# v-iashin/Synchformer

Measured on AMD Instinct MI355X. Metric: clips/sec (14-seg offset pred), higher is better.
Workload: dtype bf16; 1 GPU; BASELINE configs[1]: batched offset inference, configs/sync.yaml model (237.5M params, random-init), uint8 224x224 frames + 16 kHz waveform segments resident in HBM; RGB + log-mel front-ends and the full forward to 21-way logits inside the timed step; clips_per_gpu=16, segments=14, seg_chunk=224, hip_graph=False, parallelism=replicas x1

## Files before the change

synchformer_amd/csrc/sf_qkv_time2.hip:

```cpp
#include "sf_common.h"
#include <type_traits>
#include <stdlib.h>
#include "../../include/synchformer_hip.h"

#define QT2_NP 196
#define QT2_TP 24
#define QT2_ROWS 192
#define QT2_D 768
#define QT2_A_BYTES (QT2_ROWS * 128)
#define QT2_W_PART (128 * 128)
#define QT2_STAGE (QT2_A_BYTES + 3 * QT2_W_PART)
#ifndef QT2_ABL_HALF
#define QT2_ABL_HALF 0
#endif
#define QT2_ARR (QT2_ROWS * 128)
#define QT2_CB_OFF (6 * QT2_ARR)
#define QT2_BIAS_OFF (QT2_CB_OFF + 6 * 2048)
#define QT2_LAND_OFF (QT2_BIAS_OFF + 1536)
#define QT2_CBX_OFF QT2_CB_OFF
#define QT2_ZROW_OFF (QT2_CB_OFF + 6 * 128)
#define QT2_SC_OFF (QT2_CB_OFF + 1024)
#define QT2_SC_BYTES 2304
#define QT2_MASK_OFF (QT2_LAND_OFF + 768)
#define QT2_LDS (160 * 1024)
#define QT2_NPART 33
#ifndef QT2_ABL
#define QT2_ABL 0
#endif

struct Qt2Args {
  const bf16_t* X; int64_t ldx;
  const bf16_t* W; int64_t ldw;
  const float* bias;
  const bf16_t* side; int64_t lds_;
  bf16_t* out; int64_t ldo;
  float* cls_part;
  int64_t seq_rows;
  uint32_t n_rt;
  uint32_t pair_chunk;
  float scale;
  uint32_t stagger;
  const uint8_t* key_keep = nullptr;
  const uint8_t* sX = nullptr; int64_t ldsx = 0;
  const uint8_t* sW = nullptr; int64_t ldsw = 0;
  uint8_t* out_q = nullptr; int64_t ldq = 0; uint8_t* out_s = nullptr; int64_t splane = 0;
};
typedef __attribute__((ext_vector_type(8))) int qt2_i32x8;

typedef short qt2_s4 __attribute__((ext_vector_type(4)));
typedef __attribute__((address_space(3))) qt2_s4 qt2_lds_s4;

__device__ __forceinline__ void qt2_dma1(uint32_t voff, const void* sbase, uint32_t lds) {
  uint32_t keep;
  asm volatile("s_mov_b32 %0, m0\n\ts_mov_b32 m0, %3\n\ts_nop 0\n\tglobal_load_lds_dwordx4 %1, %2\n\ts_mov_b32 m0, %0"
               : "=&s"(keep) : "v"(voff), "s"(sbase), "s"(lds) : "memory");
}
__device__ __forceinline__ void qt2_dma_dword_addr(const void* gaddr, uint32_t lds) {
  uint32_t keep;
  asm volatile("s_mov_b32 %0, m0\n\ts_mov_b32 m0, %2\n\ts_nop 0\n\tglobal_load_lds_dword %1, off\n\ts_mov_b32 m0, %0"
               : "=&s"(keep) : "v"(gaddr), "s"(lds) : "memory");
}
template <int N>
__device__ __forceinline__ void qt2_wait_vmcnt() {
  asm volatile("" ::: "memory");
  __builtin_amdgcn_s_waitcnt((N & 0xF) | (0x7 << 4) | (0xF << 8) | ((N >> 4) << 14));
}
__device__ __forceinline__ void qt2_barrier() {
  asm volatile("" ::: "memory");
  __builtin_amdgcn_s_barrier();
  asm volatile("" ::: "memory");
}
__device__ __forceinline__ uint32_t qt2_lds_addr(const void* p) { return (uint32_t)(uintptr_t)(__attribute__((address_space(3))) const char*)p; }
__device__ __forceinline__ int qt2_arr_off(int row, int chunk) { return row * 128 + ((chunk ^ (((row >> 3) + row) & 7)) << 4); }

template <int V> using qt2_ic = std::integral_constant<int, V>;

template <bool MASK, bool MX = false>
__device__ __forceinline__ void qkv_time2_attn_body(const Qt2Args& p) {
  constexpr int ESZ = MX ? 1 : 2;
  extern __shared__ __attribute__((aligned(16))) char smem[];
  const int tid = threadIdx.x, lane = tid & 63;
  const int wave = __builtin_amdgcn_readfirstlane(tid >> 6);
  const int wm = wave >> 2, wn = wave & 3;
  const int hi = lane >> 5;

  const uint32_t xcd = blockIdx.x & 7u, li = blockIdx.x >> 3, per_xcd_blocks = gridDim.x >> 3;
  const uint32_t r8 = (p.n_rt + 7u) >> 3;
  const uint32_t rt0 = min(xcd * r8, p.n_rt), rt1 = min(rt0 + r8, p.n_rt);
  const uint32_t hc = p.pair_chunk, chunk_tiles = (rt1 - rt0) * hc, t_end = (rt1 - rt0) * 6u;
  uint32_t t = li;
  if (t >= t_end) return;
  for (uint32_t i = 0, n = ((li / hc) * 8u + xcd) * p.stagger; i < n; ++i) __builtin_amdgcn_s_sleep(32);

  uint32_t voff_a = 0, voff_w[3] = {0, 0, 0}, sc_voff = 0, cls_voff = 0;
  const int sc_seg = wave % 3;
  const int sc_lanes = sc_seg == 0 ? 48 : (sc_seg == 1 ? 64 : 32);
  const uint32_t a8 = (uint32_t)(8 * p.ldx * ESZ), w8 = (uint32_t)(8 * p.ldw * ESZ);
  const uint32_t lds0 = __builtin_amdgcn_readfirstlane(qt2_lds_addr(smem));
  const uint32_t lds_a_w = __builtin_amdgcn_readfirstlane(lds0 + wave * 3072);
  const uint32_t lds_w_w = __builtin_amdgcn_readfirstlane(lds0 + QT2_A_BYTES + wave * 2048);

  for (int x = tid; x < (MX ? 1024 : 6 * 2048) / 16; x += 512) *reinterpret_cast<uint4*>(smem + QT2_CB_OFF + x * 16) = make_uint4(0u, 0u, 0u, 0u);
  qt2_barrier();

  const char* xbase; const char* wbase;
  int64_t seq; int tb, hp;
  auto set_tile = [&](uint32_t tt) {
    const uint32_t c = tt / chunk_tiles, r = tt - c * chunk_tiles;
    const uint32_t rt = rt0 + r / hc;
    hp = (int)(c * hc + r % hc);
    seq = rt / 9u; tb = (int)(rt - (uint32_t)seq * 9u);
    xbase = reinterpret_cast<const char*>(p.X) + (seq * p.seq_rows + 1 + (int64_t)tb * QT2_TP) * p.ldx * ESZ;
    wbase = reinterpret_cast<const char*>(p.W) + (int64_t)hp * 128 * p.ldw * ESZ;
  };
  auto derive_offsets = [&]() {
    int dtid = threadIdx.x;
    asm volatile("" : "+v"(dtid));
    const int dl = dtid & 63;
    {
      const int r = wave * 3 * 8 + (dl >> 3);
      voff_a = (uint32_t)((int64_t)(wave * QT2_NP + (dl >> 3)) * p.ldx * ESZ + ((((dl & 7) ^ ((r >> 1) & 7))) << 4));
    }
#pragma unroll
    for (int j = 0; j < 3; ++j) {
      const int pr = wave * 2 * 8 + (dl >> 3);
      const int c = (pr >> 5) * 96 + j * 32 + (pr & 31);
      const int hd = c / 192, within = c - hd * 192;
      const int grow = (within >> 6) * QT2_D + hd * 64 + (within & 63);
      voff_w[j] = (uint32_t)((int64_t)grow * p.ldw * ESZ + ((((dl & 7) ^ ((pr >> 1) & 7))) << 4));
    }
    { const int ch = dl & 7, w3 = (dl >> 3) % 3, hd = (dl >> 3) / 3; cls_voff = (uint32_t)((w3 * QT2_D + hd * 64 + ch * 8) * 2); }
    if (MX) {
      if (sc_seg == 0) sc_voff = (uint32_t)((dl / 6) * QT2_NP * 4 + (dl % 6) * 16);
      else {
        const int L = (sc_seg == 1 ? 0 : 64) + dl, run = L >> 3, j = run >> 2, wnp = run & 3;
        const int c = wnp * 96 + j * 32 + (L & 7) * 4;
        const int hd = c / 192, within = c - hd * 192;
        sc_voff = (uint32_t)(((within >> 6) * QT2_D + hd * 64 + (within & 63)) * 4);
      }
    }
  };
  const uint32_t sc_lds = __builtin_amdgcn_readfirstlane(lds0 + QT2_SC_OFF + (sc_seg == 0 ? 0 : (sc_seg == 1 ? 768 : 768 + 1024)));
  auto issue_sc = [&](int kt) {
    const char* base = sc_seg == 0 ? reinterpret_cast<const char*>(p.sX) + (int64_t)kt * p.ldsx + (seq * p.seq_rows + 1 + (int64_t)tb * QT2_TP) * 4
                                   : reinterpret_cast<const char*>(p.sW) + (int64_t)kt * p.ldsw + (int64_t)hp * 512;
    if (lane < sc_lanes) qt2_dma1(sc_voff, base, sc_lds + (kt & 1) * QT2_SC_BYTES);
  };
  auto issue_a = [&](int pc, int S, int kt) {
    qt2_dma1(((pc & 1) ? (voff_a ^ 64u) : voff_a) + (uint32_t)pc * a8, xbase + kt * 128, lds_a_w + S * QT2_STAGE + pc * 1024);
  };
  auto issue_w = [&](int j, int S, int kt) {
    qt2_dma1(voff_w[j], wbase + kt * 128, lds_w_w + S * QT2_STAGE + j * QT2_W_PART);
    qt2_dma1((voff_w[j] ^ 64u) + w8, wbase + kt * 128, lds_w_w + S * QT2_STAGE + j * QT2_W_PART + 1024);
  };

  constexpr int nk = MX ? QT2_D / 128 : QT2_D / 64;
  const float sc2 = p.scale * 1.44269504088896f;
  uint32_t tcount = 0;
  auto cb_ptr = [&](int blk, int h, int row, int chunk) -> const char* {
    if (!MX) return smem + QT2_CB_OFF + (blk + h) * 2048 + qt2_arr_off(row, chunk);
    return smem + (row == 0 ? QT2_CBX_OFF + (blk + h) * 128 : QT2_ZROW_OFF) + (chunk << 4);
  };

  for (;;) {
    set_tile(t);
    const bool main_item = tb < 8;
    if (main_item) {
      derive_offsets();
      if (wave < 6) {
        if (p.bias) qt2_dma_dword_addr(p.bias + (wave % 3) * QT2_D + (hp * 2 + wave / 3) * 64 + lane, lds0 + QT2_BIAS_OFF + wave * 256);
      } else if (wave == 7) {
        if (lane < 48) qt2_dma1(cls_voff, reinterpret_cast<const char*>(p.side + seq * 33 * p.lds_ + hp * 128), lds0 + QT2_LAND_OFF);
      }
      if (MX) issue_sc(0);
      issue_w(0, 0, 0); issue_a(0, 0, 0);
      issue_w(1, 0, 0); issue_a(1, 0, 0); issue_a(2, 0, 0);
      issue_w(2, 0, 0);
      issue_w(0, 1, 1); issue_a(0, 1, 1);
      qt2_wait_vmcnt<5>();
      qt2_barrier();

      f32x16 acc[3][3];
      {
        const float* bs = reinterpret_cast<const float*>(smem + QT2_BIAS_OFF);
#pragma unroll
        for (int j = 0; j < 3; ++j)
#pragma unroll
          for (int g = 0; g < 4; ++g) {
            const float4 b4 = p.bias ? *reinterpret_cast<const float4*>(bs + wn * 96 + j * 32 + g * 8 + hi * 4) : make_float4(0.f, 0.f, 0.f, 0.f);
#pragma unroll
            for (int i = 0; i < 3; ++i) { acc[j][i][g * 4 + 0] = b4.x; acc[j][i][g * 4 + 1] = b4.y; acc[j][i][g * 4 + 2] = b4.z; acc[j][i][g * 4 + 3] = b4.w; }
          }
      }
      {
        int fo[4], fs_x = 0, fs_w = 0, shi = 0;
        {
          int ptid = threadIdx.x;
          asm volatile("" : "+v"(ptid));
          const int pl31 = ptid & 31, phi = (ptid & 63) >> 5;
#pragma unroll
          for (int kk = 0; kk < 4; ++kk) fo[kk] = pl31 * 128 + (((kk * 2 + phi) ^ ((pl31 >> 1) & 7)) << 4);
          if (MX) { fs_x = QT2_SC_OFF + (wm * 96 + pl31) * 4; fs_w = QT2_SC_OFF + 768 + (wn * 32 + pl31) * 4; shi = phi * 8; }
        }
        const int a_base = wm * 96 * 128, w_base = QT2_A_BYTES + wn * 32 * 128;
        union Qt2Frag { bf16x8 h[2]; qt2_i32x8 v; };
        Qt2Frag xf[3][2], wf[2];
        uint32_t sx[3] = {0u, 0u, 0u}, sw = 0u;
        auto read_w = [&](const char* st, int j, int par) {
#pragma unroll
          for (int kk = 0; kk < 4; ++kk) wf[kk >> 1].h[kk & 1] = *reinterpret_cast<const bf16x8*>(st + w_base + j * QT2_W_PART + fo[kk]);
          if (MX) sw = *reinterpret_cast<const uint32_t*>(smem + fs_w + j * 512 + par * QT2_SC_BYTES) >> shi;
        };
        auto mma = [&](auto Jc) {
          constexpr int J = decltype(Jc)::value;
          __builtin_amdgcn_s_setprio(1);
          if constexpr (MX) {
#pragma unroll
            for (int k2 = 0; k2 < 2; ++k2) {
#pragma unroll
              for (int i = 0; i < 3; ++i) {
                if (k2 == 0) acc[J][i] = __builtin_amdgcn_mfma_scale_f32_32x32x64_f8f6f4(wf[0].v, xf[i][0].v, acc[J][i], 0 , 0 , 0, (int)sw, 0, (int)sx[i]);
                else acc[J][i] = __builtin_amdgcn_mfma_scale_f32_32x32x64_f8f6f4(wf[1].v, xf[i][1].v, acc[J][i], 0, 0, 2, (int)sw, 2, (int)sx[i]);
              }
            }
          } else
          if (!(QT2_ABL & 2)) {
#pragma unroll
            for (int kk = 0; kk < 4; ++kk)
#pragma unroll
              for (int i = 0; i < 3; ++i) acc[J][i] = __builtin_amdgcn_mfma_f32_32x32x16_bf16(wf[kk >> 1].h[kk & 1], xf[i][kk >> 1].h[kk & 1], acc[J][i], 0, 0, 0);
          } else asm volatile("" :: "v"(wf[0].v), "v"(wf[1].v), "v"(xf[0][0].v), "v"(xf[2][1].v));
          asm volatile("" : "+v"(acc[J][0]), "+v"(acc[J][1]), "+v"(acc[J][2]));
          __builtin_amdgcn_s_setprio(0);
        };
        auto ktile = [&](auto Sc, int kt, bool ld1, bool ld2) {
          constexpr int S = decltype(Sc)::value;
          const char* st = smem + S * QT2_STAGE;
#pragma unroll
          for (int i = 0; i < 3; ++i)
#pragma unroll
            for (int kk = 0; kk < 4; ++kk) xf[i][kk >> 1].h[kk & 1] = *reinterpret_cast<const bf16x8*>(st + a_base + i * 4096 + fo[kk]);
          read_w(st, 0, S);
          if (MX) {
#pragma unroll
            for (int i = 0; i < 3; ++i) sx[i] = *reinterpret_cast<const uint32_t*>(smem + fs_x + i * 128 + S * QT2_SC_BYTES) >> shi;
          }
          __builtin_amdgcn_sched_barrier(0);
          if (ld1) { issue_w(1, S ^ 1, kt + 1); issue_a(1, S ^ 1, kt + 1); issue_a(2, S ^ 1, kt + 1); }
          qt2_barrier();
          __builtin_amdgcn_sched_barrier(0);
          mma(qt2_ic<0>{});
          __builtin_amdgcn_sched_barrier(0);
          qt2_barrier();
          read_w(st, 1, S);
          __builtin_amdgcn_sched_barrier(0);
          if (ld1) { if (MX) issue_sc(kt + 1); issue_w(2, S ^ 1, kt + 1); if (MX) qt2_wait_vmcnt<10>(); else qt2_wait_vmcnt<9>(); } else qt2_wait_vmcnt<0>();
          qt2_barrier();
          __builtin_amdgcn_sched_barrier(0);
          mma(qt2_ic<1>{});
          __builtin_amdgcn_sched_barrier(0);
          qt2_barrier();
          read_w(st, 2, S);
          __builtin_amdgcn_sched_barrier(0);
          if (ld2) { issue_w(0, S, kt + 2); issue_a(0, S, kt + 2); qt2_wait_vmcnt<5>(); }
          else if (ld1) qt2_wait_vmcnt<2>();
          else qt2_wait_vmcnt<0>();
          qt2_barrier();
          __builtin_amdgcn_sched_barrier(0);
          mma(qt2_ic<2>{});
          __builtin_amdgcn_sched_barrier(0);
          qt2_barrier();
        };
        if (wm == 1) qt2_barrier();
#pragma unroll 1
        for (int kt = 0; kt < nk; kt += 2) {
          ktile(qt2_ic<0>{}, kt, true, kt + 2 < nk);
          ktile(qt2_ic<1>{}, kt + 1, kt + 2 < nk, kt + 3 < nk);
        }
        if (wm == 0) qt2_barrier();
      }

      {
        int etid = threadIdx.x;
        asm volatile("" : "+v"(etid));
        const int el31 = etid & 31, ehi = (etid & 63) >> 5;
        uint8_t kflag = 1;
        if (MASK && etid < QT2_ROWS + 1) {
          const int fr = etid / QT2_TP, pl = etid - fr * QT2_TP;
          kflag = etid == QT2_ROWS ? p.key_keep[seq * p.seq_rows] : p.key_keep[seq * p.seq_rows + 1 + (int64_t)fr * QT2_NP + tb * QT2_TP + pl];
        }
        int rowp[3];
#pragma unroll
        for (int i = 0; i < 3; ++i) { const int R = wm * 96 + i * 32 + el31, fr = R / QT2_TP; rowp[i] = (R - fr * QT2_TP) * 8 + fr; }
#pragma unroll
        for (int j = 0; j < 3; ++j) {
          const int cb = (wn * 3 + j) * 32;
          const int hd = cb / 192, within = cb - hd * 192, which = within >> 6, feat0 = within & 63;
          const int arr = hd * 3 * QT2_ARR + (which == 1 ? 0 : (which == 2 ? QT2_ARR : 2 * QT2_ARR));
#pragma unroll
          for (int i = 0; i < 3; ++i) {
#pragma unroll
            for (int g = 0; g < 4; ++g) {
              uint2 w;
              w.x = pack_bf2(acc[j][i][g * 4 + 0], acc[j][i][g * 4 + 1]);
              w.y = pack_bf2(acc[j][i][g * 4 + 2], acc[j][i][g * 4 + 3]);
#if QT2_ABL_HALF
              *reinterpret_cast<uint2*>(smem + arr + qt2_arr_off(rowp[i], (feat0 >> 3) + g) + (ehi ^ ((el31 >> 3) & 1)) * 8) = w;
#else
              *reinterpret_cast<uint2*>(smem + arr + qt2_arr_off(rowp[i], (feat0 >> 3) + g) + ehi * 8) = w;
#endif
            }
          }
        }
        if (etid < 48) {
          const int ch = etid & 7, w3 = (etid >> 3) % 3, hd = (etid >> 3) / 3;
          const uint4 sv = *reinterpret_cast<const uint4*>(smem + QT2_LAND_OFF + etid * 16);
          *reinterpret_cast<uint4*>(const_cast<char*>(cb_ptr(w3 == 1 ? 0 : (w3 == 2 ? 2 : 4), hd, 0, ch))) = sv;
        }
        if (MASK && etid < QT2_ROWS + 1) {
          const int fr = etid / QT2_TP, pl = etid - fr * QT2_TP;
          reinterpret_cast<float*>(smem + QT2_MASK_OFF)[etid == QT2_ROWS ? QT2_ROWS : pl * 8 + fr] = kflag ? 0.f : -INFINITY;
        }
        qt2_barrier();
      }
    } else {
      int stid = threadIdx.x;
      asm volatile("" : "+v"(stid));
      uint4 sv[3], cv = make_uint4(0u, 0u, 0u, 0u);
#pragma unroll
      for (int e = 0; e < 3; ++e) {
        const int x = stid + e * 512, ch = x & 7, rr = (x >> 3) & 31, w3 = (x >> 8) % 3, hd = (x >> 8) / 3;
        sv[e] = *reinterpret_cast<const uint4*>(p.side + (seq * 33 + 1 + (rr & 7) * 4 + (rr >> 3)) * p.lds_ + w3 * QT2_D + (hp * 2 + hd) * 64 + ch * 8);
      }
      if (stid < 48) {
        const int ch = stid & 7, w3 = (stid >> 3) % 3, hd = (stid >> 3) / 3;
        cv = *reinterpret_cast<const uint4*>(p.side + seq * 33 * p.lds_ + w3 * QT2_D + (hp * 2 + hd) * 64 + ch * 8);
      }
#pragma unroll
      for (int e = 0; e < 3; ++e) {
        const int x = stid + e * 512, ch = x & 7, rr = (x >> 3) & 31, w3 = (x >> 8) % 3, hd = (x >> 8) / 3;
        *reinterpret_cast<uint4*>(smem + hd * 3 * QT2_ARR + (w3 == 1 ? 0 : (w3 == 2 ? QT2_ARR : 2 * QT2_ARR)) + qt2_arr_off(rr, ch)) = sv[e];
      }
      if (stid < 48) {
        const int ch = stid & 7, w3 = (stid >> 3) % 3, hd = (stid >> 3) / 3;
        *reinterpret_cast<uint4*>(const_cast<char*>(cb_ptr(w3 == 1 ? 0 : (w3 == 2 ? 2 : 4), hd, 0, ch))) = cv;
      }
      if (MASK && stid >= 64 && stid < 64 + 33) {
        const int r = stid - 64;
        const uint8_t kf = r == 32 ? p.key_keep[seq * p.seq_rows] : p.key_keep[seq * p.seq_rows + 1 + (int64_t)(r & 7) * QT2_NP + QT2_ROWS + (r >> 3)];
        reinterpret_cast<float*>(smem + QT2_MASK_OFF)[r == 32 ? QT2_ROWS : r] = kf ? 0.f : -INFINITY;
      }
      qt2_barrier();
    }

    if (!(QT2_ABL & 1)) {
      int atid = threadIdx.x;
      asm volatile("" : "+v"(atid));
      const int alane = atid & 63, fr_ = alane & 15, fg = alane >> 4;
      const int krow = fg * 4 + (fr_ >> 2), c1 = (fr_ & 3) >> 1, hb = (fr_ & 1) * 8;
      const int64_t orow0 = seq * p.seq_rows + 1 + (main_item ? tb * QT2_TP : QT2_ROWS);
      auto patch_units = [&](auto NUc, const int u0, const int ustep) {
        constexpr int NU = decltype(NUc)::value;
        const char* k_lds[NU];
        int qt[NU], hh_[NU];
        f32x4 s0[NU], s1[NU];
#pragma unroll
        for (int e = 0; e < NU; ++e) {
          const int u = u0 + e * ustep, h = u >= 12 ? 1 : 0;
          qt[e] = u - 12 * h;
          k_lds[e] = smem + h * 3 * QT2_ARR;
          hh_[e] = h;
          s0[e] = f32x4{0.f, 0.f, 0.f, 0.f}; s1[e] = f32x4{0.f, 0.f, 0.f, 0.f};
          if (MASK) {
            const float4 mk = *reinterpret_cast<const float4*>(smem + QT2_MASK_OFF + (qt[e] * 16 + fg * 4) * 4);
            s0[e] = f32x4{mk.x, mk.y, mk.z, mk.w};
            s1[e][0] = reinterpret_cast<const float*>(smem + QT2_MASK_OFF)[QT2_ROWS];
          }
        }
#pragma unroll
        for (int ks = 0; ks < 2; ++ks)
#pragma unroll
          for (int e = 0; e < NU; ++e) {
            const bf16x8 qf = *reinterpret_cast<const bf16x8*>(k_lds[e] + 2 * QT2_ARR + qt2_arr_off(qt[e] * 16 + fr_, ks * 4 + fg));
            const bf16x8 kf = *reinterpret_cast<const bf16x8*>(k_lds[e] + qt2_arr_off(qt[e] * 16 + fr_, ks * 4 + fg));
            const bf16x8 cf = *reinterpret_cast<const bf16x8*>(cb_ptr(0, hh_[e], fr_, ks * 4 + fg));
            s0[e] = __builtin_amdgcn_mfma_f32_16x16x32_bf16(kf, qf, s0[e], 0, 0, 0);
            s1[e] = __builtin_amdgcn_mfma_f32_16x16x32_bf16(cf, qf, s1[e], 0, 0, 0);
          }
        const bool own = (fg >> 1) == (fr_ >> 3);
        float m[NU], l[NU], pc[NU];
#pragma unroll
        for (int e = 0; e < NU; ++e) {
          m[e] = fg == 0 ? s1[e][0] : -INFINITY;
#pragma unroll
          for (int r = 0; r < 4; ++r) { s0[e][r] = own ? s0[e][r] : -INFINITY; m[e] = fmaxf(m[e], s0[e][r]); }
        }
#pragma unroll
        for (int e = 0; e < NU; ++e) m[e] = fmaxf(m[e], __shfl_xor(m[e], 16, 64));
#pragma unroll
        for (int e = 0; e < NU; ++e) {
          m[e] = fmaxf(m[e], __shfl_xor(m[e], 32, 64)) * sc2;
          if (MASK && m[e] == -INFINITY) m[e] = 0.f;
        }
#pragma unroll
        for (int e = 0; e < NU; ++e) {
          l[e] = 0.f;
#pragma unroll
          for (int r = 0; r < 4; ++r) { s0[e][r] = __builtin_amdgcn_exp2f(fmaf(s0[e][r], sc2, -m[e])); l[e] += s0[e][r]; }
          pc[e] = fg == 0 ? __builtin_amdgcn_exp2f(fmaf(s1[e][0], sc2, -m[e])) : 0.f;
          l[e] += pc[e];
        }
#pragma unroll
        for (int e = 0; e < NU; ++e) l[e] += __shfl_xor(l[e], 16, 64);
#pragma unroll
        for (int e = 0; e < NU; ++e) l[e] += __shfl_xor(l[e], 32, 64);
        f32x4 o[NU][4];
#pragma unroll
        for (int e = 0; e < NU; ++e) {
          union { bf16x8 v; uint32_t u[4]; } pa;
          pa.u[0] = pack_bf2(s0[e][0], s0[e][1]); pa.u[1] = pack_bf2(s0[e][2], s0[e][3]);
          pa.u[2] = pack_bf2(pc[e], 0.f); pa.u[3] = 0u;
#pragma unroll
          for (int dt = 0; dt < 4; ++dt) {
            union { bf16x8 v; qt2_s4 hh[2]; } vb;
            vb.hh[0] = __builtin_amdgcn_ds_read_tr16_b64_v4i16((qt2_lds_s4*)(k_lds[e] + QT2_ARR + qt2_arr_off(qt[e] * 16 + krow, dt * 2 + c1) + hb));
            vb.hh[1] = __builtin_amdgcn_ds_read_tr16_b64_v4i16((qt2_lds_s4*)(cb_ptr(2, hh_[e], krow, dt * 2 + c1) + hb));
            o[e][dt] = __builtin_amdgcn_mfma_f32_16x16x32_bf16(vb.v, pa.v, f32x4{0.f, 0.f, 0.f, 0.f}, 0, 0, 0);
          }
        }
#ifndef QT2_OUT_LINES
#define QT2_OUT_LINES 1
#endif
#pragma unroll
        for (int e = 0; e < NU; ++e) {
          const int u = u0 + e * ustep, head = hp * 2 + (u >= 12 ? 1 : 0);
          const float linv = 1.0f / l[e];
          if (QT2_OUT_LINES) {
            char* qrows = const_cast<char*>(k_lds[e]) + 2 * QT2_ARR;
#pragma unroll
            for (int dt = 0; dt < 4; ++dt) {
              uint2 w;
              w.x = pack_bf2(o[e][dt][0] * linv, o[e][dt][1] * linv);
              w.y = pack_bf2(o[e][dt][2] * linv, o[e][dt][3] * linv);
              *reinterpret_cast<uint2*>(qrows + qt2_arr_off(qt[e] * 16 + fr_, dt * 2 + (fg >> 1)) + (fg & 1) * 8) = w;
            }
          } else {
            bf16_t* orow = p.out + (orow0 + (int64_t)(fr_ & 7) * QT2_NP + 2 * qt[e] + (fr_ >> 3)) * p.ldo + head * 64 + fg * 4;
#pragma unroll
            for (int dt = 0; dt < 4; ++dt) {
              uint2 w;
              w.x = pack_bf2(o[e][dt][0] * linv, o[e][dt][1] * linv);
              w.y = pack_bf2(o[e][dt][2] * linv, o[e][dt][3] * linv);
              if (!(QT2_ABL & 32) || linv == 12345.678f) *reinterpret_cast<uint2*>(orow + dt * 16) = w;
            }
          }
        }
        if (QT2_OUT_LINES) {
#pragma unroll
          for (int e = 0; e < NU; ++e) {
            const int u = u0 + e * ustep, head = hp * 2 + (u >= 12 ? 1 : 0);
            const char* qrows = k_lds[e] + 2 * QT2_ARR;
#pragma unroll
            for (int j = 0; j < 2; ++j) {
              const int rr = (alane >> 3) + 8 * j, ch = alane & 7;
              const uint4 w = *reinterpret_cast<const uint4*>(qrows + qt2_arr_off(qt[e] * 16 + rr, ch));
              if (MX && p.out_q) {
                const int64_t row = orow0 + (int64_t)(alane >> 3) * QT2_NP + 2 * qt[e] + j;
                float fv[8];
                fv[0] = __uint_as_float(w.x << 16); fv[1] = __uint_as_float(w.x & 0xffff0000u); fv[2] = __uint_as_float(w.y << 16); fv[3] = __uint_as_float(w.y & 0xffff0000u);
                fv[4] = __uint_as_float(w.z << 16); fv[5] = __uint_as_float(w.z & 0xffff0000u); fv[6] = __uint_as_float(w.w << 16); fv[7] = __uint_as_float(w.w & 0xffff0000u);
                float amax = fmaxf(fmaxf(fmaxf(fabsf(fv[0]), fabsf(fv[1])), fmaxf(fabsf(fv[2]), fabsf(fv[3]))), fmaxf(fmaxf(fabsf(fv[4]), fabsf(fv[5])), fmaxf(fabsf(fv[6]), fabsf(fv[7]))));
                amax = fmaxf(amax, __shfl_xor(amax, 1, 64)); amax = fmaxf(amax, __shfl_xor(amax, 2, 64));
                const int be = sf_mx_exp(amax);
                const float inv = sf_mx_inv(be);
                uint2 d; d.x = sf_fp8x4(fv, inv); d.y = sf_fp8x4(fv + 4, inv);
                const int be_hi = __shfl_xor(be, 4, 64);
                if (!(QT2_ABL & 32) || l[e] == 12345.678f) {
                  *reinterpret_cast<uint2*>(p.out_q + row * p.ldq + head * 64 + ch * 8) = d;
                  if (ch == 0) *reinterpret_cast<uint16_t*>(p.out_s + (int64_t)(head >> 1) * p.splane + row * 4 + (head & 1) * 2) = (uint16_t)(be | (be_hi << 8));
                }
                continue;
              }
              bf16_t* dst = p.out + (orow0 + (int64_t)(alane >> 3) * QT2_NP + 2 * qt[e] + j) * p.ldo + head * 64 + ch * 8;
#ifndef QT2_OUT_NT
#define QT2_OUT_NT 1
#endif
              if (!(QT2_ABL & 32) || l[e] == 12345.678f) {
                typedef unsigned int qt2_u4 __attribute__((ext_vector_type(4)));
                const qt2_u4 wv = {w.x, w.y, w.z, w.w};
                if (QT2_OUT_NT) __builtin_nontemporal_store(wv, reinterpret_cast<qt2_u4*>(dst)); else *reinterpret_cast<qt2_u4*>(dst) = wv;
              }
            }
          }
        }
      };
      auto cls_unit = [&](auto NKc, auto WCc, const int h, const int kt0, const int rec) {
        constexpr int NK = decltype(NKc)::value;
        constexpr bool WITH_CLS = decltype(WCc)::value != 0;
        constexpr int NKT = NK + (WITH_CLS ? 1 : 0);
        const int head = hp * 2 + h;
        const char* k_lds = smem + h * 3 * QT2_ARR;
        const char* v_lds = k_lds + QT2_ARR;
        bf16x8 qf[2];
#pragma unroll
        for (int ks = 0; ks < 2; ++ks) qf[ks] = *reinterpret_cast<const bf16x8*>(cb_ptr(4, h, fr_, ks * 4 + fg));
        f32x4 s[NKT];
#pragma unroll
        for (int kt = 0; kt < NKT; ++kt) {
          s[kt] = f32x4{0.f, 0.f, 0.f, 0.f};
          if (MASK) {
            if (kt < NK) { const float4 mk = *reinterpret_cast<const float4*>(smem + QT2_MASK_OFF + ((kt0 + kt) * 16 + fg * 4) * 4); s[kt] = f32x4{mk.x, mk.y, mk.z, mk.w}; }
            else s[kt][0] = reinterpret_cast<const float*>(smem + QT2_MASK_OFF)[QT2_ROWS];
          }
#pragma unroll
          for (int ks = 0; ks < 2; ++ks) {
            const bf16x8 kf = kt < NK ? *reinterpret_cast<const bf16x8*>(k_lds + qt2_arr_off((kt0 + kt) * 16 + fr_, ks * 4 + fg))
                                      : *reinterpret_cast<const bf16x8*>(cb_ptr(0, h, fr_, ks * 4 + fg));
            s[kt] = __builtin_amdgcn_mfma_f32_16x16x32_bf16(kf, qf[ks], s[kt], 0, 0, 0);
          }
        }
        if (WITH_CLS) {
#pragma unroll
          for (int r = 0; r < 4; ++r)
            if (fg != 0 || r != 0) s[NKT - 1][r] = -INFINITY;
        }
        float m = -INFINITY;
#pragma unroll
        for (int kt = 0; kt < NKT; ++kt)
#pragma unroll
          for (int r = 0; r < 4; ++r) m = fmaxf(m, s[kt][r]);
        m = fmaxf(m, __shfl_xor(m, 16, 64)); m = fmaxf(m, __shfl_xor(m, 32, 64));
        const float msc = m * sc2;
        const float msafe = (MASK && m == -INFINITY) ? 0.f : msc;
        float l = 0.f;
#pragma unroll
        for (int kt = 0; kt < NKT; ++kt)
#pragma unroll
          for (int r = 0; r < 4; ++r) { const float e = __builtin_amdgcn_exp2f(fmaf(s[kt][r], sc2, -msafe)); s[kt][r] = e; l += e; }
        l += __shfl_xor(l, 16, 64); l += __shfl_xor(l, 32, 64);
        f32x4 o[4];
#pragma unroll
        for (int dt = 0; dt < 4; ++dt) o[dt] = f32x4{0.f, 0.f, 0.f, 0.f};
#pragma unroll
        for (int kk = 0; kk < (NKT + 1) / 2; ++kk) {
          union { bf16x8 v; uint32_t u[4]; } pa;
          pa.u[0] = pack_bf2(s[2 * kk][0], s[2 * kk][1]);
          pa.u[1] = pack_bf2(s[2 * kk][2], s[2 * kk][3]);
          if (2 * kk + 1 < NKT) {
            const int t1 = 2 * kk + 1 < NKT ? 2 * kk + 1 : 0;
            pa.u[2] = pack_bf2(s[t1][0], s[t1][1]);
            pa.u[3] = pack_bf2(s[t1][2], s[t1][3]);
          } else { pa.u[2] = 0u; pa.u[3] = 0u; }
#pragma unroll
          for (int dt = 0; dt < 4; ++dt) {
            union { bf16x8 v; qt2_s4 hh[2]; } vb;
            const int ta = 2 * kk, tb_ = 2 * kk + 1;
            vb.hh[0] = ta < NK ? __builtin_amdgcn_ds_read_tr16_b64_v4i16((qt2_lds_s4*)(v_lds + qt2_arr_off((kt0 + ta) * 16 + krow, dt * 2 + c1) + hb))
                               : __builtin_amdgcn_ds_read_tr16_b64_v4i16((qt2_lds_s4*)(cb_ptr(2, h, krow, dt * 2 + c1) + hb));
            vb.hh[1] = qt2_s4{0, 0, 0, 0};
            if (tb_ < NKT) vb.hh[1] = tb_ < NK ? __builtin_amdgcn_ds_read_tr16_b64_v4i16((qt2_lds_s4*)(v_lds + qt2_arr_off((kt0 + tb_) * 16 + krow, dt * 2 + c1) + hb))
                                               : __builtin_amdgcn_ds_read_tr16_b64_v4i16((qt2_lds_s4*)(cb_ptr(2, h, krow, dt * 2 + c1) + hb));
            o[dt] = __builtin_amdgcn_mfma_f32_16x16x32_bf16(vb.v, pa.v, o[dt], 0, 0, 0);
          }
        }
        if (fr_ == 0) {
          float* part = p.cls_part + ((seq * 12 + head) * QT2_NPART + rec) * 66;
          if (fg == 0) { part[0] = msc; part[1] = l; }
#pragma unroll
          for (int dt = 0; dt < 4; ++dt)
#pragma unroll
            for (int r = 0; r < 4; ++r) part[2 + dt * 16 + fg * 4 + r] = o[dt][r];
        }
      };
      const int wr = (wave + (int)tcount) & 7;
      if (main_item) {
        if (!(QT2_ABL & 8)) patch_units(qt2_ic<3>{}, wr, 8);
        if (!(QT2_ABL & 4)) cls_unit(qt2_ic<3>{}, qt2_ic<0>{}, wr & 1, 3 * (wr >> 1), tb * 4 + (wr >> 1));
      } else if (!(QT2_ABL & 16)) {
        if (wr < 2) cls_unit(qt2_ic<2>{}, qt2_ic<1>{}, wr, 0, 32);
        else if (wr < 6) { const int u = (wr - 2) & 1; patch_units(qt2_ic<1>{}, ((wr - 2) >> 1) * 12 + u, 0); }
      }
    }
    qt2_barrier();
    t += per_xcd_blocks;
    ++tcount;
    if (t >= t_end) break;
  }
}

__global__ __launch_bounds__(512, 2) void qkv_time2_attn_kernel(Qt2Args p) { qkv_time2_attn_body<false>(p); }
__global__ __launch_bounds__(512, 2) void qkv_time2_attn_masked_kernel(Qt2Args p) { qkv_time2_attn_body<true>(p); }
__global__ __launch_bounds__(512, 2) void qkv_time2_attn_mx_kernel(Qt2Args p) { qkv_time2_attn_body<false, true>(p); }

static int qt2_launch(const uint16_t* X, int64_t ldx, const uint16_t* W, int64_t ldw, const float* bias, const uint16_t* side, int64_t lds_,
                      uint16_t* out, int64_t ldo, float* cls_partial, int64_t n_seq, int n_tok, float scale, const uint8_t* key_keep, void* stream) {
  SF_CHECK_ARG(X && W && side && out && cls_partial, "sf_qkv_time_attention2: null pointer");
  SF_CHECK_ARG(n_tok == QT2_NP, "sf_qkv_time_attention2: built for 196 patches per frame (8 frames per sequence), got %d", n_tok);
  SF_CHECK_ARG((ldx % 64) == 0 && (ldw % 64) == 0 && (lds_ % 8) == 0 && (ldo % 8) == 0 && ldx >= QT2_D && ldw >= QT2_D && lds_ >= 3 * QT2_D && ldo >= QT2_D,
               "sf_qkv_time_attention2: bad row strides (ldx / ldw multiples of 64 elements)");
  SF_CHECK_ARG(((uintptr_t)X % 16) == 0 && ((uintptr_t)W % 16) == 0 && ((uintptr_t)side % 16) == 0 && ((uintptr_t)out % 16) == 0 && (!bias || ((uintptr_t)bias % 16) == 0) &&
                   ((uintptr_t)cls_partial % 8) == 0, "sf_qkv_time_attention2: operands must be 16-byte aligned");
  SF_CHECK_ARG((const void*)X != (const void*)out, "sf_qkv_time_attention2: out must not alias X");
  if (n_seq <= 0) return 0;
  const int64_t seq_rows = 1 + 8 * (int64_t)QT2_NP;
  SF_CHECK_ARG(seq_rows * ldx * 2 < ((int64_t)1 << 32) && (int64_t)3 * QT2_D * ldw * 2 < ((int64_t)1 << 32) && (int64_t)33 * lds_ * 2 < ((int64_t)1 << 32),
               "sf_qkv_time_attention2: a sequence of X, W and a sequence's side rows must stay below 4 GiB (32-bit lane offsets)");
  SF_CHECK_ARG(n_seq * 9 * 6 < ((int64_t)1 << 31), "sf_qkv_time_attention2: too many tiles");
  if (int rc = sf_prepare_kernel(key_keep ? (const void*)qkv_time2_attn_masked_kernel : (const void*)qkv_time2_attn_kernel, QT2_LDS, "sf_qkv_time_attention2")) return rc;
  const int n_cu = sf_cu_count("sf_qkv_time_attention2");
  if (n_cu <= 0) return -1;
  Qt2Args a;
  a.X = X; a.ldx = ldx; a.W = W; a.ldw = ldw; a.bias = bias; a.side = side; a.lds_ = lds_; a.out = out; a.ldo = ldo; a.cls_part = cls_partial;
  a.seq_rows = seq_rows; a.n_rt = (uint32_t)(n_seq * 9); a.scale = scale; a.key_keep = key_keep;
  static int env_hc = -1;
  if (env_hc < 0) { const char* e = getenv("SF_QT2_PAIR_CHUNK"); env_hc = e ? atoi(e) : 6; if (env_hc < 1 || 6 % env_hc) env_hc = 6; }
  a.pair_chunk = (uint32_t)env_hc;
  static int env_st = -1;
  if (env_st < 0) { const char* e = getenv("SF_QT2_STAGGER"); env_st = e ? atoi(e) : 0; if (env_st < 0) env_st = 0; }
  a.stagger = (uint32_t)env_st;
  int64_t blocks = (n_cu / 8) * 8;
  if (blocks < 8) blocks = 8;
  const int64_t need = ((n_seq * 9 * 6 + 7) / 8) * 8;
  if (blocks > need) blocks = need;
  if (key_keep) hipLaunchKernelGGL(qkv_time2_attn_masked_kernel, dim3((unsigned)blocks), dim3(512), QT2_LDS, (hipStream_t)stream, a);
  else hipLaunchKernelGGL(qkv_time2_attn_kernel, dim3((unsigned)blocks), dim3(512), QT2_LDS, (hipStream_t)stream, a);
  SF_LAUNCH_CHECK();
  return 0;
}
extern "C" int sf_qkv_time_attention2(const uint16_t* X, int64_t ldx, const uint16_t* W, int64_t ldw, const float* bias, const uint16_t* side, int64_t lds_,
                                      uint16_t* out, int64_t ldo, float* cls_partial, int64_t n_seq, int n_tok, float scale, void* stream) {
  return qt2_launch(X, ldx, W, ldw, bias, side, lds_, out, ldo, cls_partial, n_seq, n_tok, scale, nullptr, stream);
}
extern "C" int sf_qkv_time_attention2_masked(const uint16_t* X, int64_t ldx, const uint16_t* W, int64_t ldw, const float* bias, const uint16_t* side, int64_t lds_,
                                             uint16_t* out, int64_t ldo, float* cls_partial, int64_t n_seq, int n_tok, float scale, const uint8_t* key_keep, void* stream) {
  SF_CHECK_ARG(key_keep, "sf_qkv_time_attention2_masked: null key_keep (call sf_qkv_time_attention2 for an unmasked forward)");
  return qt2_launch(X, ldx, W, ldw, bias, side, lds_, out, ldo, cls_partial, n_seq, n_tok, scale, key_keep, stream);
}

extern "C" int sf_qkv_time_attention2_mx(const uint8_t* X, int64_t ldx, const uint8_t* sX, int64_t ldsx, const uint8_t* W, int64_t ldw, const uint8_t* sW, int64_t ldsw,
                                         const float* bias, const uint16_t* side, int64_t lds_, uint16_t* out, int64_t ldo, uint8_t* out_q, int64_t ldq, uint8_t* out_s,
                                         int64_t splane, float* cls_partial, int64_t n_seq, int n_tok, float scale, void* stream) {
  SF_CHECK_ARG(X && sX && W && sW && side && cls_partial && ((out != nullptr) != (out_q != nullptr)), "sf_qkv_time_attention2_mx: null pointer (exactly one of out / out_q)");
  SF_CHECK_ARG(n_tok == QT2_NP, "sf_qkv_time_attention2_mx: built for 196 patches per frame (8 frames per sequence), got %d", n_tok);
  SF_CHECK_ARG((ldx % 128) == 0 && (ldw % 128) == 0 && ldx >= QT2_D && ldw >= QT2_D && (lds_ % 8) == 0 && lds_ >= 3 * QT2_D, "sf_qkv_time_attention2_mx: bad row strides (ldx / ldw multiples of 128 bytes)");
  SF_CHECK_ARG(((uintptr_t)X % 16) == 0 && ((uintptr_t)W % 16) == 0 && ((uintptr_t)sX % 16) == 0 && ((uintptr_t)sW % 16) == 0 && ((uintptr_t)side % 16) == 0 &&
                   (!bias || ((uintptr_t)bias % 16) == 0) && ((uintptr_t)cls_partial % 8) == 0, "sf_qkv_time_attention2_mx: operands must be 16-byte aligned");
  if (out) SF_CHECK_ARG(((uintptr_t)out % 16) == 0 && (ldo % 8) == 0 && ldo >= QT2_D, "sf_qkv_time_attention2_mx: out must be a 16-byte aligned bf16 buffer");
  if (out_q) SF_CHECK_ARG(out_s && ((uintptr_t)out_q % 8) == 0 && ((uintptr_t)out_s % 2) == 0 && (ldq % 8) == 0 && ldq >= QT2_D && out_q != X && out_s != sX,
                          "sf_qkv_time_attention2_mx: out_q (8-byte aligned, ldq %% 8 == 0) / out_s must be buffers of their own");
  if (n_seq <= 0) return 0;
  const int64_t seq_rows = 1 + 8 * (int64_t)QT2_NP;
  if (out_q) SF_CHECK_ARG(splane >= n_seq * seq_rows * 4, "sf_qkv_time_attention2_mx: a scale plane holds 4 bytes per row");
  SF_CHECK_ARG((ldsx % 16) == 0 && (ldsw % 16) == 0 && ldsx >= n_seq * seq_rows * 4 && ldsw >= 3 * QT2_D * 4, "sf_qkv_time_attention2_mx: scale planes must hold one dword per row of X / W");
  SF_CHECK_ARG(seq_rows * ldx < ((int64_t)1 << 32) && (int64_t)3 * QT2_D * ldw < ((int64_t)1 << 32) && (int64_t)33 * lds_ * 2 < ((int64_t)1 << 32),
               "sf_qkv_time_attention2_mx: a sequence of X, W and a sequence's side rows must stay below 4 GiB (32-bit lane offsets)");
  SF_CHECK_ARG(n_seq * 9 * 6 < ((int64_t)1 << 31), "sf_qkv_time_attention2_mx: too many tiles");
  if (int rc = sf_prepare_kernel((const void*)qkv_time2_attn_mx_kernel, QT2_LDS, "sf_qkv_time_attention2_mx")) return rc;
  const int n_cu = sf_cu_count("sf_qkv_time_attention2_mx");
  if (n_cu <= 0) return -1;
  Qt2Args a;
  a.X = reinterpret_cast<const bf16_t*>(X); a.ldx = ldx; a.W = reinterpret_cast<const bf16_t*>(W); a.ldw = ldw; a.bias = bias; a.side = side; a.lds_ = lds_;
  a.out = out; a.ldo = ldo; a.cls_part = cls_partial; a.seq_rows = seq_rows; a.n_rt = (uint32_t)(n_seq * 9); a.scale = scale; a.pair_chunk = 6; a.stagger = 0;
  a.sX = sX; a.ldsx = ldsx; a.sW = sW; a.ldsw = ldsw; a.out_q = out_q; a.ldq = ldq; a.out_s = out_s; a.splane = splane;
  int64_t blocks = (n_cu / 8) * 8;
  if (blocks < 8) blocks = 8;
  const int64_t need = ((n_seq * 9 * 6 + 7) / 8) * 8;
  if (blocks > need) blocks = need;
  hipLaunchKernelGGL(qkv_time2_attn_mx_kernel, dim3((unsigned)blocks), dim3(512), QT2_LDS, (hipStream_t)stream, a);
  SF_LAUNCH_CHECK();
  return 0;
}
```

Baseline: 174.4 clips/s.

## Defer attention output stores to overlap with next tile's prologue loads

```diff
diff --git a/synchformer_amd/csrc/sf_qkv_time2.hip b/synchformer_amd/csrc/sf_qkv_time2.hip
--- a/synchformer_amd/csrc/sf_qkv_time2.hip
+++ b/synchformer_amd/csrc/sf_qkv_time2.hip
@@ -65,6 +65,28 @@
   asm volatile("" ::: "memory");
   __builtin_amdgcn_s_waitcnt((N & 0xF) | (0x7 << 4) | (0xF << 8) | ((N >> 4) << 14));
 }
+__device__ __forceinline__ void qt2_wait_prologue(int stores) {
+  if (stores >= 21) qt2_wait_vmcnt<26>();
+  else if (stores >= 15) qt2_wait_vmcnt<20>();
+  else if (stores >= 12) qt2_wait_vmcnt<17>();
+  else if (stores >= 9) qt2_wait_vmcnt<14>();
+  else if (stores >= 4) qt2_wait_vmcnt<9>();
+  else if (stores >= 2) qt2_wait_vmcnt<7>();
+  else qt2_wait_vmcnt<5>();
+}
+#ifndef QT2_OUT_NT
+#define QT2_OUT_NT 1
+#endif
+typedef unsigned int qt2_u4 __attribute__((ext_vector_type(4)));
+typedef unsigned int qt2_u2 __attribute__((ext_vector_type(2)));
+typedef float qt2_f2 __attribute__((ext_vector_type(2)));
+__device__ __forceinline__ void qt2_store_line(void* g, qt2_u4 v) {
+  if (QT2_OUT_NT) asm volatile("global_store_dwordx4 %0, %1, off nt\n\ts_nop 1" :: "v"(g), "v"(v) : "memory");
+  else asm volatile("global_store_dwordx4 %0, %1, off\n\ts_nop 1" :: "v"(g), "v"(v) : "memory");
+}
+__device__ __forceinline__ void qt2_store_u2(void* g, qt2_u2 v) { asm volatile("global_store_dwordx2 %0, %1, off" :: "v"(g), "v"(v) : "memory"); }
+__device__ __forceinline__ void qt2_store_f2(void* g, qt2_f2 v) { asm volatile("global_store_dwordx2 %0, %1, off" :: "v"(g), "v"(v) : "memory"); }
+__device__ __forceinline__ void qt2_store_u16(void* g, uint32_t v) { asm volatile("global_store_short %0, %1, off" :: "v"(g), "v"(v) : "memory"); }
 __device__ __forceinline__ void qt2_barrier() {
   asm volatile("" ::: "memory");
   __builtin_amdgcn_s_barrier();
@@ -162,22 +184,149 @@
     return smem + (row == 0 ? QT2_CBX_OFF + (blk + h) * 128 : QT2_ZROW_OFF) + (chunk << 4);
   };
 
-  for (;;) {
-    set_tile(t);
-    const bool main_item = tb < 8;
+  uint2 ho[3][4];
+  f32x4 hcls[4];
+  float hmsc = 0.f, hl = 0.f;
+#pragma unroll
+  for (int e = 0; e < 3; ++e)
+#pragma unroll
+    for (int dt = 0; dt < 4; ++dt) ho[e][dt] = make_uint2(0u, 0u);
+#pragma unroll
+  for (int dt = 0; dt < 4; ++dt) hcls[dt] = f32x4{0.f, 0.f, 0.f, 0.f};
+  bool f_have = false, f_main = false;
+  int64_t f_seq = 0; int f_tb = 0, f_hp = 0, f_wr = 0;
+  auto flush = [&]() -> int {
+    if (!f_have || (QT2_ABL & 1)) return 0;
+    int ftid = threadIdx.x;
+    asm volatile("" : "+v"(ftid));
+    const int flane = ftid & 63, fr_ = flane & 15, fg = flane >> 4;
+    const int64_t orow0 = f_seq * p.seq_rows + 1 + (f_main ? f_tb * QT2_TP : QT2_ROWS);
+    char* stg = smem + QT2_STAGE + QT2_A_BYTES + QT2_W_PART + wave * 4096;
+    const bool to_q = MX && p.out_q;
+    auto patch_out = [&](auto NUc, const int u0, const int ustep) -> int {
+      constexpr int NU = decltype(NUc)::value;
+#pragma unroll
+      for (int e0 = 0; e0 < NU; e0 += 2) {
+#pragma unroll
+        for (int k = 0; k < 2; ++k) {
+          const int e = e0 + k;
+          if (e >= NU) continue;
+#pragma unroll
+          for (int dt = 0; dt < 4; ++dt) *reinterpret_cast<uint2*>(stg + k * 2048 + qt2_arr_off(fr_, dt * 2 + (fg >> 1)) + (fg & 1) * 8) = ho[e][dt];
+        }
+#pragma unroll
+        for (int k = 0; k < 2; ++k) {
+          const int e = e0 + k;
+          if (e >= NU) continue;
+          const int u = u0 + e * ustep, h = u >= 12 ? 1 : 0, qt = u - 12 * h, head = f_hp * 2 + h;
+#pragma unroll
+          for (int j = 0; j < 2; ++j) {
+            const int rr = (flane >> 3) + 8 * j, ch = flane & 7;
+            const uint4 w = *reinterpret_cast<const uint4*>(stg + k * 2048 + qt2_arr_off(rr, ch));
+            const int64_t row = orow0 + (int64_t)(flane >> 3) * QT2_NP + 2 * qt + j;
+            if (to_q) {
+              float fv[8];
+              fv[0] = __uint_as_float(w.x << 16); fv[1] = __uint_as_float(w.x & 0xffff0000u); fv[2] = __uint_as_float(w.y << 16); fv[3] = __uint_as_float(w.y & 0xffff0000u);
+              fv[4] = __uint_as_float(w.z << 16); fv[5] = __uint_as_float(w.z & 0xffff0000u); fv[6] = __uint_as_float(w.w << 16); fv[7] = __uint_as_float(w.w & 0xffff0000u);
+              float amax = fmaxf(fmaxf(fmaxf(fabsf(fv[0]), fabsf(fv[1])), fmaxf(fabsf(fv[2]), fabsf(fv[3]))), fmaxf(fmaxf(fabsf(fv[4]), fabsf(fv[5])), fmaxf(fabsf(fv[6]), fabsf(fv[7]))));
+              amax = fmaxf(amax, __shfl_xor(amax, 1, 64)); amax = fmaxf(amax, __shfl_xor(amax, 2, 64));
+              const int be = sf_mx_exp(amax);
+              const float inv = sf_mx_inv(be);
+              qt2_u2 d; d.x = sf_fp8x4(fv, inv); d.y = sf_fp8x4(fv + 4, inv);
+              const int be_hi = __shfl_xor(be, 4, 64);
+              if (!(QT2_ABL & 32) || w.x == 0x12345678u) {
+                qt2_store_u2(p.out_q + row * p.ldq + head * 64 + ch * 8, d);
+                if (ch == 0) qt2_store_u16(p.out_s + (int64_t)(head >> 1) * p.splane + row * 4 + (head & 1) * 2, (uint32_t)(be | (be_hi << 8)));
+              }
+            } else if (!(QT2_ABL & 32) || w.x == 0x12345678u) {
+              qt2_store_line(p.out + row * p.ldo + head * 64 + ch * 8, qt2_u4{w.x, w.y, w.z, w.w});
+            }
+          }
+        }
+      }
+      return (QT2_ABL & 32) ? 0 : NU * (to_q ? 4 : 2);
+    };
+    auto cls_out = [&](const int h, const int rec) -> int {
+      if (fr_ == 0) {
+        float* part = p.cls_part + ((f_seq * 12 + f_hp * 2 + h) * QT2_NPART + rec) * 66;
+        if (fg == 0) qt2_store_f2(part, qt2_f2{hmsc, hl});
+#pragma unroll
+        for (int dt = 0; dt < 4; ++dt) {
+          qt2_store_f2(part + 2 + dt * 16 + fg * 4, qt2_f2{hcls[dt][0], hcls[dt][1]});
+          qt2_store_f2(part + 4 + dt * 16 + fg * 4, qt2_f2{hcls[dt][2], hcls[dt][3]});
+        }
+      }
+      return 9;
+    };
+    int n = 0;
+    if (f_main) {
+      if (!(QT2_ABL & 8)) n += patch_out(qt2_ic<3>{}, f_wr, 8);
+      if (!(QT2_ABL & 4)) n += cls_out(f_wr & 1, f_tb * 4 + (f_wr >> 1));
+    } else if (!(QT2_ABL & 16)) {
+      if (f_wr < 2) n += cls_out(f_wr, 32);
+      else if (f_wr < 6) { const int u = (f_wr - 2) & 1; n += patch_out(qt2_ic<1>{}, ((f_wr - 2) >> 1) * 12 + u, 0); }
+    }
+    return n;
+  };
+
+  bool main_item = false;
+  int pend = 0;
+  auto begin_item = [&]() {
+    main_item = tb < 8;
     if (main_item) {
       derive_offsets();
+      int btid = threadIdx.x;
+      asm volatile("" : "+v"(btid));
+      const int blane = btid & 63;
       if (wave < 6) {
-        if (p.bias) qt2_dma_dword_addr(p.bias + (wave % 3) * QT2_D + (hp * 2 + wave / 3) * 64 + lane, lds0 + QT2_BIAS_OFF + wave * 256);
+        if (p.bias) qt2_dma_dword_addr(p.bias + (wave % 3) * QT2_D + (hp * 2 + wave / 3) * 64 + blane, lds0 + QT2_BIAS_OFF + wave * 256);
       } else if (wave == 7) {
-        if (lane < 48) qt2_dma1(cls_voff, reinterpret_cast<const char*>(p.side + seq * 33 * p.lds_ + hp * 128), lds0 + QT2_LAND_OFF);
+        if (blane < 48) qt2_dma1(cls_voff, reinterpret_cast<const char*>(p.side + seq * 33 * p.lds_ + hp * 128), lds0 + QT2_LAND_OFF);
       }
       if (MX) issue_sc(0);
       issue_w(0, 0, 0); issue_a(0, 0, 0);
       issue_w(1, 0, 0); issue_a(1, 0, 0); issue_a(2, 0, 0);
       issue_w(2, 0, 0);
       issue_w(0, 1, 1); issue_a(0, 1, 1);
-      qt2_wait_vmcnt<5>();
+      pend = flush();
+    } else {
+      int stid = threadIdx.x;
+      asm volatile("" : "+v"(stid));
+      uint4 cv = make_uint4(0u, 0u, 0u, 0u);
+      auto side_src = [&](const int e) -> const uint4* {
+        const int x = stid + e * 512, ch = x & 7, rr = (x >> 3) & 31, w3 = (x >> 8) % 3, hd = (x >> 8) / 3;
+        return reinterpret_cast<const uint4*>(p.side + (seq * 33 + 1 + (rr & 7) * 4 + (rr >> 3)) * p.lds_ + w3 * QT2_D + (hp * 2 + hd) * 64 + ch * 8);
+      };
+      auto side_dst = [&](const int e) -> uint4* {
+        const int x = stid + e * 512, ch = x & 7, rr = (x >> 3) & 31, w3 = (x >> 8) % 3, hd = (x >> 8) / 3;
+        return reinterpret_cast<uint4*>(smem + hd * 3 * QT2_ARR + (w3 == 1 ? 0 : (w3 == 2 ? QT2_ARR : 2 * QT2_ARR)) + qt2_arr_off(rr, ch));
+      };
+      const uint4 sv0 = *side_src(0), sv1 = *side_src(1), sv2 = *side_src(2);
+      if (stid < 48) {
+        const int ch = stid & 7, w3 = (stid >> 3) % 3, hd = (stid >> 3) / 3;
+        cv = *reinterpret_cast<const uint4*>(p.side + seq * 33 * p.lds_ + w3 * QT2_D + (hp * 2 + hd) * 64 + ch * 8);
+      }
+      pend = flush();
+      qt2_barrier();
+      *side_dst(0) = sv0; *side_dst(1) = sv1; *side_dst(2) = sv2;
+      if (stid < 48) {
+        const int ch = stid & 7, w3 = (stid >> 3) % 3, hd = (stid >> 3) / 3;
+        *reinterpret_cast<uint4*>(const_cast<char*>(cb_ptr(w3 == 1 ? 0 : (w3 == 2 ? 2 : 4), hd, 0, ch))) = cv;
+      }
+      if (MASK && stid >= 64 && stid < 64 + 33) {
+        const int r = stid - 64;
+        const uint8_t kf = r == 32 ? p.key_keep[seq * p.seq_rows] : p.key_keep[seq * p.seq_rows + 1 + (int64_t)(r & 7) * QT2_NP + QT2_ROWS + (r >> 3)];
+        reinterpret_cast<float*>(smem + QT2_MASK_OFF)[r == 32 ? QT2_ROWS : r] = kf ? 0.f : -INFINITY;
+      }
+      qt2_barrier();
+    }
+  };
+
+  set_tile(t);
+  begin_item();
+  for (;;) {
+    if (main_item) {
+      qt2_wait_prologue(pend);
       qt2_barrier();
 
       f32x16 acc[3][3];
@@ -323,34 +472,6 @@
         }
         qt2_barrier();
       }
-    } else {
-      int stid = threadIdx.x;
-      asm volatile("" : "+v"(stid));
-      uint4 sv[3], cv = make_uint4(0u, 0u, 0u, 0u);
-#pragma unroll
-      for (int e = 0; e < 3; ++e) {
-        const int x = stid + e * 512, ch = x & 7, rr = (x >> 3) & 31, w3 = (x >> 8) % 3, hd = (x >> 8) / 3;
-        sv[e] = *reinterpret_cast<const uint4*>(p.side + (seq * 33 + 1 + (rr & 7) * 4 + (rr >> 3)) * p.lds_ + w3 * QT2_D + (hp * 2 + hd) * 64 + ch * 8);
-      }
-      if (stid < 48) {
-        const int ch = stid & 7, w3 = (stid >> 3) % 3, hd = (stid >> 3) / 3;
-        cv = *reinterpret_cast<const uint4*>(p.side + seq * 33 * p.lds_ + w3 * QT2_D + (hp * 2 + hd) * 64 + ch * 8);
-      }
-#pragma unroll
-      for (int e = 0; e < 3; ++e) {
-        const int x = stid + e * 512, ch = x & 7, rr = (x >> 3) & 31, w3 = (x >> 8) % 3, hd = (x >> 8) / 3;
-        *reinterpret_cast<uint4*>(smem + hd * 3 * QT2_ARR + (w3 == 1 ? 0 : (w3 == 2 ? QT2_ARR : 2 * QT2_ARR)) + qt2_arr_off(rr, ch)) = sv[e];
-      }
-      if (stid < 48) {
-        const int ch = stid & 7, w3 = (stid >> 3) % 3, hd = (stid >> 3) / 3;
-        *reinterpret_cast<uint4*>(const_cast<char*>(cb_ptr(w3 == 1 ? 0 : (w3 == 2 ? 2 : 4), hd, 0, ch))) = cv;
-      }
-      if (MASK && stid >= 64 && stid < 64 + 33) {
-        const int r = stid - 64;
-        const uint8_t kf = r == 32 ? p.key_keep[seq * p.seq_rows] : p.key_keep[seq * p.seq_rows + 1 + (int64_t)(r & 7) * QT2_NP + QT2_ROWS + (r >> 3)];
-        reinterpret_cast<float*>(smem + QT2_MASK_OFF)[r == 32 ? QT2_ROWS : r] = kf ? 0.f : -INFINITY;
-      }
-      qt2_barrier();
     }
 
     if (!(QT2_ABL & 1)) {
@@ -358,7 +479,13 @@
       asm volatile("" : "+v"(atid));
       const int alane = atid & 63, fr_ = alane & 15, fg = alane >> 4;
       const int krow = fg * 4 + (fr_ >> 2), c1 = (fr_ & 3) >> 1, hb = (fr_ & 1) * 8;
-      const int64_t orow0 = seq * p.seq_rows + 1 + (main_item ? tb * QT2_TP : QT2_ROWS);
+#pragma unroll
+      for (int e = 0; e < 3; ++e)
+#pragma unroll
+        for (int dt = 0; dt < 4; ++dt) ho[e][dt] = make_uint2(0u, 0u);
+#pragma unroll
+      for (int dt = 0; dt < 4; ++dt) hcls[dt] = f32x4{0.f, 0.f, 0.f, 0.f};
+      hmsc = 0.f; hl = 0.f;
       auto patch_units = [&](auto NUc, const int u0, const int ustep) {
         constexpr int NU = decltype(NUc)::value;
         const char* k_lds[NU];
@@ -428,69 +555,13 @@
             o[e][dt] = __builtin_amdgcn_mfma_f32_16x16x32_bf16(vb.v, pa.v, f32x4{0.f, 0.f, 0.f, 0.f}, 0, 0, 0);
           }
         }
-#ifndef QT2_OUT_LINES
-#define QT2_OUT_LINES 1
-#endif
 #pragma unroll
         for (int e = 0; e < NU; ++e) {
-          const int u = u0 + e * ustep, head = hp * 2 + (u >= 12 ? 1 : 0);
           const float linv = 1.0f / l[e];
-          if (QT2_OUT_LINES) {
-            char* qrows = const_cast<char*>(k_lds[e]) + 2 * QT2_ARR;
-#pragma unroll
-            for (int dt = 0; dt < 4; ++dt) {
-              uint2 w;
-              w.x = pack_bf2(o[e][dt][0] * linv, o[e][dt][1] * linv);
-              w.y = pack_bf2(o[e][dt][2] * linv, o[e][dt][3] * linv);
-              *reinterpret_cast<uint2*>(qrows + qt2_arr_off(qt[e] * 16 + fr_, dt * 2 + (fg >> 1)) + (fg & 1) * 8) = w;
-            }
-          } else {
-            bf16_t* orow = p.out + (orow0 + (int64_t)(fr_ & 7) * QT2_NP + 2 * qt[e] + (fr_ >> 3)) * p.ldo + head * 64 + fg * 4;
-#pragma unroll
-            for (int dt = 0; dt < 4; ++dt) {
-              uint2 w;
-              w.x = pack_bf2(o[e][dt][0] * linv, o[e][dt][1] * linv);
-              w.y = pack_bf2(o[e][dt][2] * linv, o[e][dt][3] * linv);
-              if (!(QT2_ABL & 32) || linv == 12345.678f) *reinterpret_cast<uint2*>(orow + dt * 16) = w;
-            }
-          }
-        }
-        if (QT2_OUT_LINES) {
-#pragma unroll
-          for (int e = 0; e < NU; ++e) {
-            const int u = u0 + e * ustep, head = hp * 2 + (u >= 12 ? 1 : 0);
-            const char* qrows = k_lds[e] + 2 * QT2_ARR;
-#pragma unroll
-            for (int j = 0; j < 2; ++j) {
-              const int rr = (alane >> 3) + 8 * j, ch = alane & 7;
-              const uint4 w = *reinterpret_cast<const uint4*>(qrows + qt2_arr_off(qt[e] * 16 + rr, ch));
-              if (MX && p.out_q) {
-                const int64_t row = orow0 + (int64_t)(alane >> 3) * QT2_NP + 2 * qt[e] + j;
-                float fv[8];
-                fv[0] = __uint_as_float(w.x << 16); fv[1] = __uint_as_float(w.x & 0xffff0000u); fv[2] = __uint_as_float(w.y << 16); fv[3] = __uint_as_float(w.y & 0xffff0000u);
-                fv[4] = __uint_as_float(w.z << 16); fv[5] = __uint_as_float(w.z & 0xffff0000u); fv[6] = __uint_as_float(w.w << 16); fv[7] = __uint_as_float(w.w & 0xffff0000u);
-                float amax = fmaxf(fmaxf(fmaxf(fabsf(fv[0]), fabsf(fv[1])), fmaxf(fabsf(fv[2]), fabsf(fv[3]))), fmaxf(fmaxf(fabsf(fv[4]), fabsf(fv[5])), fmaxf(fabsf(fv[6]), fabsf(fv[7]))));
-                amax = fmaxf(amax, __shfl_xor(amax, 1, 64)); amax = fmaxf(amax, __shfl_xor(amax, 2, 64));
-                const int be = sf_mx_exp(amax);
-                const float inv = sf_mx_inv(be);
-                uint2 d; d.x = sf_fp8x4(fv, inv); d.y = sf_fp8x4(fv + 4, inv);
-                const int be_hi = __shfl_xor(be, 4, 64);
-                if (!(QT2_ABL & 32) || l[e] == 12345.678f) {
-                  *reinterpret_cast<uint2*>(p.out_q + row * p.ldq + head * 64 + ch * 8) = d;
-                  if (ch == 0) *reinterpret_cast<uint16_t*>(p.out_s + (int64_t)(head >> 1) * p.splane + row * 4 + (head & 1) * 2) = (uint16_t)(be | (be_hi << 8));
-                }
-                continue;
-              }
-              bf16_t* dst = p.out + (orow0 + (int64_t)(alane >> 3) * QT2_NP + 2 * qt[e] + j) * p.ldo + head * 64 + ch * 8;
-#ifndef QT2_OUT_NT
-#define QT2_OUT_NT 1
-#endif
-              if (!(QT2_ABL & 32) || l[e] == 12345.678f) {
-                typedef unsigned int qt2_u4 __attribute__((ext_vector_type(4)));
-                const qt2_u4 wv = {w.x, w.y, w.z, w.w};
-                if (QT2_OUT_NT) __builtin_nontemporal_store(wv, reinterpret_cast<qt2_u4*>(dst)); else *reinterpret_cast<qt2_u4*>(dst) = wv;
-              }
-            }
+#pragma unroll
+          for (int dt = 0; dt < 4; ++dt) {
+            ho[e][dt].x = pack_bf2(o[e][dt][0] * linv, o[e][dt][1] * linv);
+            ho[e][dt].y = pack_bf2(o[e][dt][2] * linv, o[e][dt][3] * linv);
           }
         }
       };
@@ -498,7 +569,6 @@
         constexpr int NK = decltype(NKc)::value;
         constexpr bool WITH_CLS = decltype(WCc)::value != 0;
         constexpr int NKT = NK + (WITH_CLS ? 1 : 0);
-        const int head = hp * 2 + h;
         const char* k_lds = smem + h * 3 * QT2_ARR;
         const char* v_lds = k_lds + QT2_ARR;
         bf16x8 qf[2];
@@ -563,14 +633,9 @@
             o[dt] = __builtin_amdgcn_mfma_f32_16x16x32_bf16(vb.v, pa.v, o[dt], 0, 0, 0);
           }
         }
-        if (fr_ == 0) {
-          float* part = p.cls_part + ((seq * 12 + head) * QT2_NPART + rec) * 66;
-          if (fg == 0) { part[0] = msc; part[1] = l; }
-#pragma unroll
-          for (int dt = 0; dt < 4; ++dt)
-#pragma unroll
-            for (int r = 0; r < 4; ++r) part[2 + dt * 16 + fg * 4 + r] = o[dt][r];
-        }
+        hmsc = msc; hl = l;
+#pragma unroll
+        for (int dt = 0; dt < 4; ++dt) hcls[dt] = o[dt];
       };
       const int wr = (wave + (int)tcount) & 7;
       if (main_item) {
@@ -580,12 +645,16 @@
         if (wr < 2) cls_unit(qt2_ic<2>{}, qt2_ic<1>{}, wr, 0, 32);
         else if (wr < 6) { const int u = (wr - 2) & 1; patch_units(qt2_ic<1>{}, ((wr - 2) >> 1) * 12 + u, 0); }
       }
+      f_have = true; f_main = main_item; f_seq = seq; f_tb = tb; f_hp = hp; f_wr = wr;
     }
     qt2_barrier();
     t += per_xcd_blocks;
     ++tcount;
     if (t >= t_end) break;
+    set_tile(t);
+    begin_item();
   }
+  flush();
 }
 
 __global__ __launch_bounds__(512, 2) void qkv_time2_attn_kernel(Qt2Args p) { qkv_time2_attn_body<false>(p); }
```

Result: no change. 174.6 clips/s (median of 4 runs) (+0.2%).
